# IntelLabs/GKL

Hardware: AMD Instinct MI355X
Metric: pairhmm_gcups (higher is better)
Workload: dtype f32

## Files before the change

### gkl_amd/csrc/pairhmm_aux_kernels.h

```cpp
#pragma once
#include <hip/hip_runtime.h>
#include <stdint.h>

#include "../../include/gkl_hip_pairhmm.h"
#include "pairhmm_fwd_kernel.h"
#include "pairhmm_multi_sets.h"

namespace gklhip {

struct PrepArgs {
  const uint8_t* hap_bases;
  const int32_t* hap_src;
  const int32_t* hap_len;
  const int32_t* hap_pos;
  const int32_t* hap_group;
  const int32_t* hap_pos_flat;
  uint32_t* stream_flat;
  uint32_t* stream;
  uint8_t* hap_has_n;
  int32_t n_haps;
  int32_t* clear_a; int32_t n_a;
  int32_t* clear_b; int32_t n_b;
  int32_t* clear_c; int32_t n_c;
  const uint4* pull_src; uint4* pull_dst; int32_t pull_n16;
// ... 219 lines not shown
struct FinalizeArgs {
  const float* raw32;
  const double* raw64;
  double* out;
  uint8_t* used64;
  int32_t* count;
  int32_t* read_fail;
  int32_t n_haps;
  int64_t n;
  int mode;
  float log10_init_f;
  double log10_init32_as_f64;
  double log10_init_d;
};

__global__ void finalize32_kernel(FinalizeArgs a) {
  const int64_t i = (int64_t)blockIdx.x * blockDim.x + threadIdx.x;
  if (i >= a.n || a.used64[i]) return;
  const float v = a.raw32[i];
  if (a.mode == GKLHIP_FINALIZE_DEVICE_F64) a.out[i] = log10((double)v) - a.log10_init32_as_f64;
  else if (a.mode == GKLHIP_FINALIZE_DEVICE_REF32) a.out[i] = (double)((float)log10((double)v) - a.log10_init_f);
}

__global__ void finalize64_kernel(FinalizeArgs a, int all_pairs) {
  const int64_t p = (int64_t)blockIdx.x * blockDim.x + threadIdx.x;
  if (p >= a.n) return;
  if (all_pairs) a.used64[p] = 1;
  else if (!a.used64[p]) return;
  if (a.mode >= 0) a.out[p] = log10(a.raw64[p]) - a.log10_init_d;
  if (a.mode == kModePacked) reinterpret_cast<uint64_t*>(a.out)[p] = packed_word(a.raw64[p]);
}

#ifndef GKL_PACK_WINDOW
#define GKL_PACK_WINDOW 96
#endif
constexpr int kPackWindow = GKL_PACK_WINDOW;
// ... 13 lines not shown
  LaneSlot* lanes2;
  const int32_t* hap_orig;
  const int32_t* hap_group;
  const int32_t* hap_pos;
  const int32_t* hap_len;
  FwdJob* jobs;
  FwdJob* sorted;
  const LaneSlot* long_lanes;
  int32_t n_long;
  FwdJob* jobs_long;
  int32_t* long_chunk_jobs;
  int32_t total_cols;
  int32_t wanted_jobs;
  int32_t min_job_cols;
  int32_t packed_by_kernels;
};

__device__ __forceinline__ bool last_block_done(int32_t* arrivals) {
  __shared__ int32_t s_is_last;
  __syncthreads();
  if (threadIdx.x == 0) {
    __threadfence();
    const int32_t before = atomicAdd(arrivals, 1);
    s_is_last = before == (int32_t)gridDim.x - 1 ? 1 : 0;
    __threadfence();
  }
  __syncthreads();
  return s_is_last != 0;
}

__device__ __forceinline__ int32_t ld_cnt(int32_t* p) { return __hip_atomic_load(p, __ATOMIC_RELAXED, __HIP_MEMORY_SCOPE_AGENT); }

__device__ __forceinline__ int job_class(const FwdJob& j, const int32_t* hap_pos, const int32_t* hap_len) {
  const int cols = hap_pos[j.hap_end - 1] + hap_len[j.hap_end - 1] - hap_pos[j.hap_begin];
  const int c = cols >> 7;
  return kJobClasses - 1 - (c < kJobClasses - 1 ? c : kJobClasses - 1);
}

__device__ __forceinline__ void build_jobs_for_chunk(const PlanArgs& a, const LaneSlot* lanes, int c, FwdJob* jobs,
                                                     int32_t* chunk_jobs, int cut_cols, bool by_group, int lane) {
  const LaneSlot sl = lanes[(int64_t)c * kLanes + lane];
  jobs += (int64_t)c * a.n_haps;
  int n_jobs = 0;
  bool prev_need = false;
  uint64_t reads = __ballot(sl.read >= 0 && sl.block == 0);
  for (int k0 = 0; k0 < a.n_haps; k0 += kLanes) {
    const int k = k0 + lane;
    const bool in = k < a.n_haps;
    const int h = in ? a.hap_orig[k] : 0;
    uint8_t nd = 0;
    for (uint64_t m = reads; m; m &= m - 1) {
      const int r = __builtin_amdgcn_readlane(sl.read, __builtin_ctzll(m));
      if (in) nd |= a.fa.used64[(int64_t)r * a.n_haps + h];
    }
    const uint64_t need = __ballot(in && nd != 0);
    if (!need) { prev_need = false; continue; }
    bool start = false;
    if (in && nd) {
      const bool pred_needed = lane == 0 ? prev_need : ((need >> (lane - 1)) & 1ull) != 0;
      start = !pred_needed || a.hap_pos[k - 1] / cut_cols != a.hap_pos[k] / cut_cols ||
              (by_group && a.hap_group[k - 1] != a.hap_group[k]);
    }
    const uint64_t starts = __ballot(start);
    if ((need & 1ull) && !(starts & 1ull)) {
      const uint64_t stop = starts | ~need;
      const int e = stop ? __builtin_ctzll(stop) : kLanes;
      if (lane == 0) jobs[n_jobs - 1].hap_end = min(k0 + e, a.n_haps);
    }
    const int base = n_jobs;
    n_jobs += __builtin_popcountll(starts);
    if (start) {
      const uint64_t after = lane == kLanes - 1 ? 0ull : (~0ull << (lane + 1));
      const uint64_t stop = (starts | ~need) & after;
      const int e = stop ? __builtin_ctzll(stop) : kLanes;
      FwdJob j;
      j.chunk = c; j.hap_begin = k; j.hap_end = min(k0 + e, a.n_haps);
      j.klass = 0;
      jobs[base + __builtin_popcountll(starts & ((1ull << lane) - 1ull))] = j;
    }
    prev_need = ((need >> (kLanes - 1)) & 1ull) != 0;
  }
  __threadfence_block();
  for (int i = lane; i < n_jobs; i += kLanes) {
    FwdJob j = jobs[i];
    jobs[i].klass = job_class(j, a.hap_pos, a.hap_len);
  }
  if (lane == 0) chunk_jobs[c] = n_jobs;
}

#define GKLHIP_PLAN_STAMP(k) do { if (tid == 0) a.cnts[16 + (k)] = (int32_t)(wall_clock64() - clk0); } while (0)

constexpr int kPlanLdsBins = 4096;
template <bool kInLds>
__device__ __forceinline__ void order_affected_reads(const PlanArgs& a, int32_t* hist, int32_t* pos, int32_t* s_wave_tot,
                                                     int tid, uint64_t clk0) {
  constexpr int kBatch = 4;
  const int n = a.n_haps, lane = tid & 63, wave = tid >> 6;
  if (kInLds) {
    for (int c = tid; c < n + 2; c += kPlanBlock) hist[c] = 0;
    __syncthreads();
  }
// ... 73 lines not shown
      const bool fails = in_range && v < 1e-28f;
      const uint64_t mask = __ballot(fails);
      if (mask) {
        const int leader = __builtin_ctzll(mask);
        const int32_t read = fails ? (int32_t)((uint32_t)i / (uint32_t)a.n_haps) : -1;
        const int32_t lead_read = __shfl(read, leader, 64);
        const uint64_t same = __ballot(fails && read == lead_read);
        if (lane == leader) atomicAdd(a.fa.read_fail + lead_read, __builtin_popcountll(same));
        if (fails && read != lead_read) atomicAdd(a.fa.read_fail + read, 1);
        if (lane == 0) my_fails += __builtin_popcountll(mask);
      }
      if (in_range) {
        a.fa.used64[i] = fails ? 1 : 0;
        if (a.fa.mode == kModePacked && !a.packed_by_kernels)
          reinterpret_cast<uint64_t*>(a.fa.out)[i] = fails ? 0ull : (kPackedF32Tag | (uint64_t)__float_as_uint(v));
      }
    }
    if (lane == 0) s_wave[wave] = my_fails;
    __syncthreads();
    if (tid == 0) {
      int total = 0;
      for (int w = 0; w < kPlanBlock / 64; w++) total += s_wave[w];
      if (total) atomicAdd(a.cnts + 0, total);
    }
  }
  if (!last_block_done(a.cnts + 10)) return;
  const int n_fail = ld_cnt(a.cnts + 0);
  if (n_fail == 0) return;
  const uint64_t clk0 = wall_clock64();

  if (a.n_haps + 2 <= kPlanLdsBins) order_affected_reads<true>(a, s_hist, s_hist + kPlanLdsBins, s_i32, tid, clk0);
  else                             order_affected_reads<false>(a, a.hist, a.pos, s_i32, tid, clk0);
  GKLHIP_PLAN_STAMP(2);
}

__global__ __launch_bounds__(kPlanBlock) void plan_pack_kernel(PlanArgs a) {
  const int tid = (int)threadIdx.x, lane = tid & 63, wave = tid >> 6;
  const int nblk = (int)gridDim.x, blk = (int)blockIdx.x;
  if (ld_cnt(a.cnts + 0) == 0) return;
  const uint64_t clk0 = wall_clock64();

  {
    static_assert(kPackWindow <= 2 * kLanes, "the window's lane counts sit in two registers per lane");
    __shared__ int32_t s_pack[kPlanBlock / 64][4][kPackWindow];
    int32_t* s_read = s_pack[wave][0]; int32_t* s_needl = s_pack[wave][1]; int32_t* s_sread = s_pack[wave][2];
    int32_t* s_sneed = s_pack[wave][3];
    const int n = ld_cnt(a.cnts + 4);
    const int n_win = (n + kPackWindow - 1) / kPackWindow;
    for (int w = blk * (kPlanBlock / 64) + wave; w < n_win; w += nblk * (kPlanBlock / 64)) {
      const int w0 = w * kPackWindow;
      const int cnt = min(kPackWindow, n - w0);
      for (int i = lane; i < cnt; i += kLanes) {
        const int r = a.order[w0 + i];
        s_read[i] = r;
        s_needl[i] = (int)((a.read_off[r + 1] - a.read_off[r] + a.rpl) / a.rpl);
      }
      __builtin_amdgcn_wave_barrier();
      if (w == 0 && lane == 0) a.cnts[22] = (int32_t)(wall_clock64() - clk0);
      for (int i = lane; i < cnt; i += kLanes) {
        const int ni = s_needl[i];
        int rank = 0;
        for (int j = 0; j < cnt; j++) {
          const int nj = s_needl[j];
          rank += (nj > ni) || (nj == ni && j < i);
        }
        s_sread[rank] = s_read[i];
        s_sneed[rank] = ni;
      }
      __builtin_amdgcn_wave_barrier();
      if (w == 0 && lane == 0) a.cnts[23] = (int32_t)(wall_clock64() - clk0);
      int head = -1, next_lo = -1, next_hi = -1;
      int bin_lo = 0, off_lo = 0, bin_hi = 0, off_hi = 0;
      uint64_t avail = 0;
      int nb = 0;
      const int need_lo = lane < cnt ? s_sneed[lane] : 0, need_hi = lane + kLanes < cnt ? s_sneed[lane + kLanes] : 0;
      for (int i = 0; i < cnt; i++) {
        const int nn = __builtin_amdgcn_readlane(i < kLanes ? need_lo : need_hi, i & 63);
        const uint64_t fits = nn >= kLanes ? 0ull : (avail >> nn) << nn;
        int bin, f;
        if (fits) {
          f = __builtin_ctzll(fits);
          bin = __builtin_amdgcn_readlane(head, f);
          const int nxt = __builtin_amdgcn_readlane(bin < kLanes ? next_lo : next_hi, bin & 63);
          if (lane == f) head = nxt;
          if (nxt < 0) avail &= ~(1ull << f);
        } else {
          bin = nb++;
          f = kLanes;
        }
        const int left = f - nn;
        if (left > 0) {
          const int old = __builtin_amdgcn_readlane(head, left);
          if (lane == (bin & 63)) { if (bin < kLanes) next_lo = old; else next_hi = old; }
          if (lane == left) head = bin;
          avail |= 1ull << left;
        }
        if (lane == (i & 63)) { if (i < kLanes) { bin_lo = bin; off_lo = kLanes - f; } else { bin_hi = bin; off_hi = kLanes - f; } }
      }
      if (w == 0 && lane == 0) a.cnts[24] = (int32_t)(wall_clock64() - clk0);
      int base = 0;
      if (lane == 0) base = atomicAdd(a.cnts + 5, nb);
      base = __shfl(base, 0, kLanes);
      LaneSlot idle; idle.read = -1; idle.block = 0;
      for (int i = lane; i < nb * kLanes; i += kLanes) a.lanes2[(int64_t)base * kLanes + i] = idle;
      __builtin_amdgcn_wave_barrier();
      __threadfence_block();
      if (w == 0 && lane == 0) a.cnts[25] = (int32_t)(wall_clock64() - clk0);
      if (lane < cnt) {
        LaneSlot sl; sl.read = s_sread[lane];
        LaneSlot* dst = a.lanes2 + (int64_t)(base + bin_lo) * kLanes + off_lo;
        for (int b = 0; b < need_lo; b++) { sl.block = b; dst[b] = sl; }
      }
      if (lane + kLanes < cnt) {
        LaneSlot sl; sl.read = s_sread[lane + kLanes];
        LaneSlot* dst = a.lanes2 + (int64_t)(base + bin_hi) * kLanes + off_hi;
        for (int b = 0; b < need_hi; b++) { sl.block = b; dst[b] = sl; }
      }
      __builtin_amdgcn_wave_barrier();
      if (w == 0 && lane == 0) a.cnts[26] = (int32_t)(wall_clock64() - clk0);
    }
  }
  if (blk == 0) GKLHIP_PLAN_STAMP(3);
}

__global__ __launch_bounds__(kPlanBlock) void plan_jobs_kernel(PlanArgs a) {
  __shared__ int32_t s_i32[kPlanBlock];
  const int tid = (int)threadIdx.x, lane = tid & 63, wave = tid >> 6;
  const int nblk = (int)gridDim.x, blk = (int)blockIdx.x;
  const int n_fail = ld_cnt(a.cnts + 0);
  if (n_fail == 0) return;
  const uint64_t clk0 = wall_clock64();

  {
    const int total = ld_cnt(a.cnts + 5);
    const int n_fail_reads = ld_cnt(a.cnts + 4);
    const double density = (double)n_fail / ((double)max(n_fail_reads, 1) * (double)a.n_haps);
    const double est_steps = (double)max(total, 1) * (double)a.total_cols * fmin(density, 1.0);
    const int cut_cols = max(a.min_job_cols, (int)fmin(est_steps / (double)a.wanted_jobs, 1e9));
    const int n_waves = nblk * (kPlanBlock / 64), w = blk * (kPlanBlock / 64) + wave;
    for (int c = w; c < total; c += n_waves) build_jobs_for_chunk(a, a.lanes2, c, a.jobs, a.order, cut_cols, false, lane);
    for (int c = w; c < a.n_long; c += n_waves) build_jobs_for_chunk(a, a.long_lanes, c, a.jobs_long, a.long_chunk_jobs, 0x7fffffff, true, lane);
  }
  if (!last_block_done(a.cnts + 11)) return;
  GKLHIP_PLAN_STAMP(4);

  {
    int32_t* cnt = s_i32;
    int32_t* base = s_i32 + kJobClasses;
    const int total = ld_cnt(a.cnts + 5);
    __syncthreads();
    if (tid < kJobClasses) cnt[tid] = 0;
    __syncthreads();
    for (int c = tid; c < total; c += kPlanBlock) {
      const FwdJob* mine = a.jobs + (int64_t)c * a.n_haps;
      const int n = a.order[c];
      for (int i = 0; i < n; i++) atomicAdd(&cnt[mine[i].klass], 1);
    }
    __syncthreads();
    if (tid == 0) {
      int acc = 0;
      for (int c = 0; c < kJobClasses; c++) { base[c] = acc; acc += cnt[c]; }
      a.cnts[2] = acc;
    }
    __syncthreads();
    for (int c = tid; c < total; c += kPlanBlock) {
      const FwdJob* mine = a.jobs + (int64_t)c * a.n_haps;
      const int n = a.order[c];
      for (int i = 0; i < n; i++) {
        const FwdJob j = mine[i];
        a.sorted[atomicAdd(&base[j.klass], 1)] = j;
      }
    }
    if (tid == 0 && a.n_long > 0) {
      int at = 0;
      for (int c = 0; c < a.n_long; c++) {
        const int n = a.long_chunk_jobs[c];
        for (int i = 0; i < n; i++) a.jobs_long[at++] = a.jobs_long[(int64_t)c * a.n_haps + i];
      }
      a.cnts[8] = at;
    }
  }
  GKLHIP_PLAN_STAMP(5);
}
#undef GKLHIP_PLAN_STAMP

// ... 223 lines not shown
```

### gkl_amd/csrc/pairhmm_ctx.h

```cpp
#pragma once

using namespace gklhip;

namespace {
struct EnvSwitches {
  static bool on_unless_zero(const char* name) { const char* v = getenv(name); return !v || atoi(v) != 0; }
  static int integer(const char* name) { const char* v = getenv(name); return v ? atoi(v) : 0; }
  const bool wide_long = on_unless_zero("GKLHIP_WIDE_LONG");
  const bool super_long = on_unless_zero("GKLHIP_SUPER_LONG");
  const bool fused_pairs = on_unless_zero("GKLHIP_FUSED_PAIRS");
  const int64_t fused_max = [] { const char* v = getenv("GKLHIP_FUSED_MAX_PAIRS"); return v ? atoll(v) : -1LL; }();
  const bool xcd_aware = on_unless_zero("GKLHIP_XCD_AWARE");
  const bool timing = getenv("GKLHIP_TIMING") != nullptr;
  const int combine_load = integer("GKL_HIP_COMBINE_LOAD");
  const int target_cols = integer("GKLHIP_TARGET_COLS");
  const int fb_wanted_jobs = integer("GKLHIP_FB_WANTED_JOBS");
  const int plan_blocks = integer("GKLHIP_PLAN_BLOCKS");
  const int finalize_threads = integer("GKL_HIP_FINALIZE_THREADS");
  const int finalize_min = integer("GKL_HIP_FINALIZE_MIN");
  const bool combine = [] { const char* v = getenv("GKL_HIP_COMBINE"); return !(v && v[0] == '0'); }();
  const bool combine_mid = integer("GKL_HIP_COMBINE_MID") != 0;
  const bool quiet = getenv("GKL_HIP_QUIET") != nullptr;
  const bool one_device_engine = integer("GKL_HIP_DEVICE_ENGINES") == 1;
  const int small_read_limit = integer("GKL_HIP_SMALL_READ_LIMIT") == 511 ? 511 : 383;
// ... 21 lines not shown
  PinBuf stage_slot[2];
  DevBuf plan_dev_slot[2];
  hipEvent_t stage_free_slot[2] = {nullptr, nullptr};
  hipEvent_t plan_unused_slot[2] = {nullptr, nullptr};
  hipStream_t upload_stream = nullptr;
  bool upload_eager = false;
  hipStream_t pad_stream = nullptr;
  int plan_slot = 0;
  DevBuf raw32, raw64, used64, counters, stream_buf, out_dev;
  DevBuf lanes_main;
  DevBuf read_fail, lanes2, jobs, jobs_long, fail_order, fail_hist, hap_flags;
  DevBuf batch_dev;
  PinBuf res_pin;
  WorkerPool workers;
  hipStream_t copy_stream = nullptr;
  hipEvent_t policy_done = nullptr, early_copy_done = nullptr;
  hipEvent_t call_done = nullptr;
  bool have_call_done = false;
  static constexpr int kEventRing = 64;
  hipEvent_t ev_ring[kEventRing][6] = {};
  hipEvent_t* ev = ev_ring[0];
  int64_t calls = 0;
  bool ring_double[kEventRing] = {};
  gklhip_stats stats;
  int64_t last_pairs = 0;
  hipStream_t last_stream = nullptr;
  bool have_last = false;
  Plan plan;
  std::vector<PlanLane> long_lanes;
  std::vector<FwdJob> long_jobs;
  DevBuf carry;
// ... 4 lines not shown
```

### gkl_amd/csrc/pairhmm_ctx_lifecycle.h

```cpp
#pragma once

namespace {

std::atomic<int> g_eager_upload_holders{0};

int trim_streams(DevCtx* c) {
  if (!c->copy_stream && !c->pad_stream && (!c->upload_stream || c->upload_eager)) return 0;
  (void)hipSetDevice(c->device);
  for (hipStream_t s : {c->stream, c->copy_stream, c->upload_stream, c->have_last ? c->last_stream : nullptr})
    if (s && hipStreamQuery(s) != hipSuccess) { (void)hipGetLastError(); return 0; }
  int n = 0;
  if (c->copy_stream) { (void)hipStreamDestroy(c->copy_stream); c->copy_stream = nullptr; n++; }
  if (c->pad_stream) { (void)hipStreamDestroy(c->pad_stream); c->pad_stream = nullptr; n++; }
  if (c->upload_stream && !c->upload_eager) { (void)hipStreamDestroy(c->upload_stream); c->upload_stream = nullptr; n++; }
  return n;
}

void dev_done(DevCtx* c) {
  if (!c) return;
  (void)hipSetDevice(c->device);
  if (c->upload_eager) g_eager_upload_holders--;
  if (c->stream) (void)hipStreamSynchronize(c->stream);
  if (c->last_stream && c->have_last) (void)hipStreamSynchronize(c->last_stream);
  for (DevBuf* b : {&c->tab32, &c->tab64, &c->plan_dev_slot[0], &c->plan_dev_slot[1], &c->raw32, &c->raw64, &c->used64,
                    &c->counters, &c->stream_buf, &c->out_dev, &c->batch_dev, &c->read_fail, &c->lanes_main,
                    &c->lanes2, &c->jobs, &c->jobs_long, &c->fail_order, &c->fail_hist, &c->carry, &c->hap_flags})
    b->release();
  c->stage_slot[0].release();
  c->stage_slot[1].release();
  c->res_pin.release();
  c->multi_fallbacks.release();
  if (c->multi_in) (void)hipEventDestroy(c->multi_in);
  if (c->policy_done) (void)hipEventDestroy(c->policy_done);
  if (c->early_copy_done) (void)hipEventDestroy(c->early_copy_done);
  if (c->call_done) (void)hipEventDestroy(c->call_done);
  if (c->copy_stream) { (void)hipStreamSynchronize(c->copy_stream); (void)hipStreamDestroy(c->copy_stream); }
  for (auto& set : c->ev_ring)
    for (auto& e : set) if (e) (void)hipEventDestroy(e);
  for (int k = 0; k < 2; k++) {
    if (c->stage_free_slot[k]) (void)hipEventDestroy(c->stage_free_slot[k]);
    if (c->plan_unused_slot[k]) (void)hipEventDestroy(c->plan_unused_slot[k]);
  }
  if (c->upload_stream) { (void)hipStreamSynchronize(c->upload_stream); (void)hipStreamDestroy(c->upload_stream); }
  if (c->pad_stream) (void)hipStreamDestroy(c->pad_stream);
  if (c->stream) (void)hipStreamDestroy(c->stream);
  delete c;
}

int dev_init(const gklhip_config& cfg, int dev, int ndev, DevCtx** out) {
// ... 73 lines not shown
    if (hipStreamCreateWithFlags(&c->upload_stream, hipStreamNonBlocking) != hipSuccess) { g_eager_upload_holders--; return bail(fail(GKLHIP_ERR_HIP, "hipStreamCreate failed")); }
    c->upload_eager = true;
  } else {
    g_eager_upload_holders--;
  }
  if (const char* v = getenv("GKL_HIP_EAGER_STREAMS")) {
    const int k = atoi(v);
    if (k >= 7) { if (aux_streams(c) != GKLHIP_OK) return bail(GKLHIP_ERR_HIP); }
    else for (int i = 0; i < k; i++) { hipStream_t d = nullptr; (void)hipStreamCreateWithFlags(&d, hipStreamNonBlocking); }
  }
  for (int k = 0; k < 2; k++)
    if (hipEventCreateWithFlags(&c->stage_free_slot[k], hipEventDisableTiming) != hipSuccess ||
        hipEventCreateWithFlags(&c->plan_unused_slot[k], hipEventDisableTiming) != hipSuccess)
      return bail(fail(GKLHIP_ERR_HIP, "hipEventCreate failed"));
  if (hipEventCreateWithFlags(&c->policy_done, hipEventDisableTiming) != hipSuccess ||
      hipEventCreateWithFlags(&c->early_copy_done, hipEventDisableTiming) != hipSuccess ||
      hipEventCreateWithFlags(&c->call_done, hipEventDisableTiming) != hipSuccess)
    return bail(fail(GKLHIP_ERR_HIP, "hipEventCreate failed"));
  for (int k = 0; k < 2; k++)
    if (hipEventRecord(c->stage_free_slot[k], c->stream) != hipSuccess || hipEventRecord(c->plan_unused_slot[k], c->stream) != hipSuccess)
      return bail(fail(GKLHIP_ERR_HIP, "hipEventRecord failed"));
  {
    const int sets = c->cfg.record_events == 2 ? DevCtx::kEventRing : 1;
    for (int k = 0; k < sets; k++)
      for (auto& e : c->ev_ring[k])
        if (hipEventCreate(&e) != hipSuccess) return bail(fail(GKLHIP_ERR_HIP, "hipEventCreate failed"));
  }
  if ((rc = upload_tables(c, host_tables_f32(), &c->tab32, &c->dt32))) return bail(rc);
  if ((rc = upload_tables(c, host_tables_f64(), &c->tab64, &c->dt64))) return bail(rc);
  *out = c;
  return GKLHIP_OK;
// ... 42 lines not shown
```

### gkl_amd/csrc/pairhmm_device_pass.h

```cpp
#pragma once

namespace {

int aux_streams(DevCtx* c) {
  if (!c->upload_stream) HIP_TRY(hipStreamCreateWithFlags(&c->upload_stream, hipStreamNonBlocking));
  if (!c->copy_stream) {
    HIP_TRY(hipStreamCreateWithFlags(&c->copy_stream, hipStreamNonBlocking));
    if (!c->pad_stream) HIP_TRY(hipStreamCreateWithFlags(&c->pad_stream, hipStreamNonBlocking));
  }
  return GKLHIP_OK;
}

template <typename T>
int upload_tables(DevCtx* c, const HostTables<T>& h, DevBuf* buf, DevTables<T>* dt) {
  const size_t n = (size_t)kQuals * 2 + kMmEntries;
  int st = buf->reserve(n * sizeof(T));
  if (st) return st;
  T* base = buf->as<T>();
  {
    T* pin = nullptr;
    HIP_TRY(hipHostMalloc(reinterpret_cast<void**>(&pin), n * sizeof(T), hipHostMallocDefault));
    memcpy(pin, h.ph2pr.data(), kQuals * sizeof(T));
    memcpy(pin + kQuals, h.div3.data(), kQuals * sizeof(T));
    memcpy(pin + 2 * kQuals, h.mm.data(), kMmEntries * sizeof(T));
// ... 135 lines not shown
};

#ifndef GKL_RPL_F64
#define GKL_RPL_F64 6
#endif
constexpr int kRplF64 = GKL_RPL_F64;
#ifndef GKL_RPL_F64_JOBS
#define GKL_RPL_F64_JOBS 10
#endif
constexpr int kRplF64Jobs = GKL_RPL_F64_JOBS;
constexpr int kRplF64Wide = 8;
constexpr size_t kSmallBatchBytes = 1 << 20;
constexpr int64_t kDirectPairs = 65536;
constexpr int64_t kTwoStepFrom = 2048;
constexpr int64_t kSmallDoublePairs = kTwoStepFrom;
constexpr int kPlanBlocks = 64;
constexpr int kFallbackWantedJobs = 12288;
constexpr int64_t kHostShardPairs = 400000;
constexpr int64_t kOnePassPairs = 65536;
constexpr int kTargetCols = 2048;
#ifndef GKL_RPL_F32
#define GKL_RPL_F32 8
#endif
constexpr int kRplF32 = GKL_RPL_F32;
std::atomic<int> g_host_calls_in_flight{0};
int pick_f32_rpl(int forced, int n_reads, int n_haps, const int64_t* read_off, const int64_t* hap_off, int load = 1) {
  int max_len = 0;
  for (int r = 0; r < n_reads; r++) max_len = std::max(max_len, (int)(read_off[r + 1] - read_off[r]));
  if (forced == 2 && max_len <= 2 * kLanes - 1) return 2;
  if (forced == 4 || forced == -4 || forced == 2) return 4;
  if (forced == 8) return kRplF32;
// ... 299 lines not shown
  } else {
    if ((rc = aux_streams(c))) return rc;
    HIP_TRY(hipStreamWaitEvent(c->upload_stream, c->plan_unused_slot[slot], 0));
    HIP_TRY(hipMemcpyAsync(dp, hs, L.total, hipMemcpyHostToDevice, c->upload_stream));
    HIP_TRY(hipEventRecord(c->stage_free_slot[slot], c->upload_stream));
    HIP_TRY(hipStreamWaitEvent(s, c->stage_free_slot[slot], 0));
  }
  if (g_env.timing)
    fprintf(stderr, "[gklhip] host plan + staging: %.3f ms (%d chunks, %d stream entries, %zu plan bytes)\n",
            std::chrono::duration<double, std::milli>(std::chrono::steady_clock::now() - P.t0).count(),
            plan.n_chunks, plan.n_stream, L.total);

  if ((rc = c->raw32.reserve((size_t)P.n_pairs * 4))) return rc;
  if ((rc = c->raw64.reserve((size_t)P.n_pairs * 8))) return rc;
  if ((rc = c->used64.reserve((size_t)P.n_pairs))) return rc;
  if ((rc = c->counters.reserve(128))) return rc;
  if ((rc = c->read_fail.reserve((size_t)P.n_reads * 4))) return rc;
  if ((rc = c->stream_buf.reserve(((size_t)plan.n_stream + (size_t)plan.n_stream_flat) * 4))) return rc;
  if (!P.use_double && (rc = c->fail_hist.reserve((size_t)P.n_hist * 4))) return rc;
  if ((rc = c->hap_flags.reserve((size_t)P.n_haps))) return rc;
  if ((rc = c->lanes_main.reserve((size_t)std::max(plan.n_chunks, 1) * kLanes * sizeof(LaneSlot)))) return rc;

  S.s = s; S.out = out_dev; S.slot = slot; S.hs = hs; S.dp = dp; S.xcarry = nullptr;
  const gklhip_batch dbi = P.inline_host() ? batch_at(*db, dp + L.batch, L.batch_stride) : *db;
  S.b = DevBatch{dbi.read_bases, dbi.read_quals, dbi.ins_gop, dbi.del_gop, dbi.gcp, reinterpret_cast<const int64_t*>(dp + L.read_off), P.n_reads, P.n_haps};
  S.hap_bases = (P.pull && P.inline_host()) ? batch_at(*db, S.hs_dev + L.batch, L.batch_stride).hap_bases : dbi.hap_bases;
  S.stream_grouped = P.inline_host() ? reinterpret_cast<uint32_t*>(dp + L.stream) : c->stream_buf.as<uint32_t>();
  S.stream_flat = P.inline_host() ? reinterpret_cast<uint32_t*>(dp + L.stream_flat) : c->stream_buf.as<uint32_t>() + plan.n_stream;
  S.hap_has_n = P.inline_host() ? dp + L.has_n : c->hap_flags.as<uint8_t>();
  return GKLHIP_OK;
}
// ... 117 lines not shown
  pa.lanes2 = c->lanes2.as<LaneSlot>();
  pa.hap_orig = reinterpret_cast<const int32_t*>(dp + L.hap_orig);
  pa.hap_group = reinterpret_cast<const int32_t*>(dp + L.hap_group);
  pa.hap_pos = reinterpret_cast<const int32_t*>(dp + L.hap_pos_flat);
  pa.hap_len = reinterpret_cast<const int32_t*>(dp + L.hap_len);
  pa.jobs = c->jobs.as<FwdJob>();
  pa.sorted = c->jobs.as<FwdJob>() + planned_max_jobs(P);
  pa.long_lanes = reinterpret_cast<const LaneSlot*>(dp + L.long_lanes) + (size_t)P.n_long_main * kLanes;
  pa.n_long = P.n_long64;
  pa.jobs_long = c->jobs_long.as<FwdJob>();
  pa.long_chunk_jobs = c->fail_order.as<int32_t>() + n_reads;
  pa.total_cols = (int32_t)std::min<int64_t>((int64_t)P.hl + n_haps, 0x7fffffff);
  pa.wanted_jobs = g_env.fb_wanted_jobs > 0 ? g_env.fb_wanted_jobs : (int)std::min<int64_t>(kFallbackWantedJobs, std::max<int64_t>(4096, P.n_pairs / 100));
  pa.min_job_cols = 256;
  pa.packed_by_kernels = (P.finalize_mode == kModePacked && !P.per_pair) ? 1 : 0;
  return pa;
}

int launch_prep(DevCtx* c, const CallPlan& P, const StagedCall& S) {
  const bool ev = c->cfg.record_events != 0;
  if (ev) {
    const bool deferred = c->cfg.record_events == 2;
    c->ev = c->ev_ring[deferred ? c->calls % DevCtx::kEventRing : 0];
    c->ring_double[deferred ? c->calls % DevCtx::kEventRing : 0] = P.use_double;
    c->calls++;
    HIP_TRY(hipEventRecord(c->ev[0], S.s));
  }
  const PrepArgs pa = prep_args(c, P, S);
  hipLaunchKernelGGL(prep_kernel, dim3((unsigned)prep_grid(pa, P)), dim3(kPrepBlock), 0, S.s, pa);
  if (P.pull) HIP_TRY(hipEventRecord(c->stage_free_slot[S.slot], S.s));
// ... 51 lines not shown
int launch_planned_fp64(DevCtx* c, const CallPlan& P, const StagedCall& S) {
  const bool ev = c->cfg.record_events != 0;
  hipStream_t s = S.s;
  const int n_reads = P.n_reads;
  const int64_t n_pairs = P.n_pairs;
  const size_t max_jobs = planned_max_jobs(P);
  int rc;
  if ((rc = c->fail_order.reserve(((size_t)n_reads + (size_t)P.n_long64) * 4))) return rc;
  if ((rc = c->lanes2.reserve((size_t)n_reads * kLanes * sizeof(LaneSlot)))) return rc;
  if ((rc = c->jobs.reserve(2 * max_jobs * sizeof(FwdJob)))) return rc;
  if (P.n_long64 > 0 && (rc = c->jobs_long.reserve((size_t)P.n_long64 * (size_t)P.n_haps * sizeof(FwdJob)))) return rc;
  const PlanArgs pa = plan_args(c, P, S);
  const int blocks_env = g_env.plan_blocks;
  const int policy_grid = std::max(1, blocks_env > 0 ? blocks_env : (int)std::min<int64_t>(c->n_cus, std::max<int64_t>(16, n_pairs / 4096)));
  const int64_t max_windows = ((int64_t)n_reads + kPackWindow - 1) / kPackWindow;
  const int pack_grid = (int)std::max<int64_t>(1, std::min<int64_t>(kPlanBlocks, (max_windows + kPlanBlock / 64 - 1) / (kPlanBlock / 64)));
  const int jobs_grid = std::max(1, std::min(c->n_cus, blocks_env > 0 ? blocks_env : (int)std::min<int64_t>(kPlanBlocks, std::max<int64_t>(16, n_pairs / 8192))));
  hipLaunchKernelGGL(plan_policy_kernel, dim3((unsigned)policy_grid), dim3(kPlanBlock), 0, s, pa);
  HIP_TRY(hipEventRecord(c->policy_done, s));
  hipLaunchKernelGGL(plan_pack_kernel, dim3((unsigned)pack_grid), dim3(kPlanBlock), 0, s, pa);
  hipLaunchKernelGGL(plan_jobs_kernel, dim3((unsigned)jobs_grid), dim3(kPlanBlock), 0, s, pa);
  const bool side_finalize = finalizes_on_device(P.finalize_mode);
  if (side_finalize) {
    if ((rc = aux_streams(c))) return rc;
    HIP_TRY(hipStreamWaitEvent(c->copy_stream, c->policy_done, 0));
    hipLaunchKernelGGL(finalize32_kernel, dim3((unsigned)((n_pairs + 255) / 256)), dim3(256), 0, c->copy_stream, pa.fa);
    HIP_TRY(hipEventRecord(c->early_copy_done, c->copy_stream));
  }
  FwdArgs<double> d = recompute_args(c, P, S);
  d.chunk_lanes = c->lanes2.as<LaneSlot>();
  d.n_chunks = n_reads;
  d.jobs = c->jobs.as<FwdJob>() + max_jobs;
  if (ev) HIP_TRY(hipEventRecord(c->ev[3], s));
  launch_jobs<double, kRplF64Jobs>(d, P.fma, (int)std::min<int64_t>(n_pairs, (int64_t)c->n_cus * 16), s);
  if (P.n_long64 > 0) {
    int32_t* cnts = c->counters.as<int32_t>();
    FwdArgs<double> ld = d;
    ld.chunk_lanes = pa.long_lanes;
    ld.jobs = c->jobs_long.as<FwdJob>();
    ld.job_count = cnts + 8;
    ld.job_next = cnts + 9;
    launch_long_jobs<double, kRplF64Wide, kRplF64>(ld, P.fma, P.n_long_waves, c->plan.max_read_len, c->carry.as<double>(), P.carry_len, s, S.xcarry, P.xsteps, cnts + 13);
  }
  if (ev) HIP_TRY(hipEventRecord(c->ev[4], s));
  hipLaunchKernelGGL(finalize64_kernel, dim3((unsigned)((n_pairs + 255) / 256)), dim3(256), 0, s, pa.fa, 0);
  if (side_finalize) HIP_TRY(hipStreamWaitEvent(s, c->early_copy_done, 0));
  return GKLHIP_OK;
}
int finish_call(DevCtx* c, const CallPlan& P, const StagedCall& S) {
  const bool ev = c->cfg.record_events != 0;
  hipStream_t s = S.s;
  gklhip_stats& st = c->stats;
  if (ev) HIP_TRY(hipEventRecord(c->ev[5], s));
  HIP_TRY(hipGetLastError());

  HIP_TRY(hipEventRecord(c->plan_unused_slot[S.slot], s));
  HIP_TRY(hipEventRecord(c->call_done, s));
  c->have_call_done = true;
  c->last_pairs = P.n_pairs;
  c->last_stream = s;
  c->have_last = true;

  if (ev && c->cfg.record_events != 2) {
    HIP_TRY(hipEventSynchronize(c->ev[5]));
    float ms = 0;
    HIP_TRY(hipEventElapsedTime(&ms, c->ev[1], c->ev[2])); st.ms_fwd_main = ms;
    HIP_TRY(hipEventElapsedTime(&ms, c->ev[3], c->ev[4])); st.ms_fwd_fallback = P.use_double ? 0.f : ms;
    HIP_TRY(hipEventElapsedTime(&ms, c->ev[0], c->ev[5])); st.ms_total_device = ms;
    int32_t cnt[2] = {0, 0};
    HIP_TRY(hipMemcpyAsync(cnt, c->counters.p, 8, hipMemcpyDeviceToHost, s));
    HIP_TRY(hipStreamSynchronize(s));
    st.n_fallback = P.use_double ? P.n_pairs : cnt[0];
    if (g_env.timing && !P.use_double) {
      int32_t k[32];
      HIP_TRY(hipMemcpy(k, c->counters.p, sizeof k, hipMemcpyDeviceToHost));
      fprintf(stderr, "[gklhip] policy+plan phases, each from the start of its own launch (us): hist %.1f scan %.1f scatter %.1f pack %.1f jobs %.1f sort %.1f | "
              "%d affected reads, %d chunks, %d jobs | window 0: loaded %.1f ranked %.1f fitted %.1f cleared %.1f written %.1f\n",
              k[16] * 0.01, k[17] * 0.01, k[18] * 0.01, k[19] * 0.01, k[20] * 0.01, k[21] * 0.01,
              k[4], k[5], k[2], k[22] * 0.01, k[23] * 0.01, k[24] * 0.01, k[25] * 0.01, k[26] * 0.01);
    }
  } else {
    st.n_fallback = P.use_double ? P.n_pairs : -1;
  }
  return GKLHIP_OK;
}

int32_t small_call_kind(const CallPlan& P) {
  if (P.use_double && P.n_pairs > kSmallDoublePairs) return kSmallDoubleStream;
  return P.pair_double ? kSmallDouble : P.fused ? kSmallFused : P.n_pairs > kTwoStepFrom ? kSmallTwoStep : kSmallOneLaunch;
}
bool small_kind_is_mid(int32_t kind) { return kind == kSmallTwoStep || kind == kSmallDoubleStream; }

void describe_small_call(DevCtx* c, const CallPlan& P, const StagedCall& S, SmallLaunch* out) {
  SmallCall& k = out->call;
// ... 49 lines not shown
```

Before: 4669.

## Fuse f32 finalize into policy kernel and restructure fallback planning kernels

Drops the separate finalize32 kernel and its side stream, event wait and pass over the pairs by writing the f32 log10 result inside the policy kernel. Job classes are now computed as each job is stored and counted per block, so the jobs kernel merges per-block class counts instead of re-reading every job to build a histogram. The pack kernel moves to 256-thread blocks with a larger grid, ranks two window entries per lane, and makes bin placement branch-free. It also batches the flag reads in build_jobs and the job loads in the scatter, at the cost of more code complexity and an extra per-block counter buffer.

```diff
diff --git a/gkl_amd/csrc/pairhmm_aux_kernels.h b/gkl_amd/csrc/pairhmm_aux_kernels.h
--- a/gkl_amd/csrc/pairhmm_aux_kernels.h
+++ b/gkl_amd/csrc/pairhmm_aux_kernels.h
@@ -257,12 +257,9 @@
   double log10_init_d;
 };
 
-__global__ void finalize32_kernel(FinalizeArgs a) {
-  const int64_t i = (int64_t)blockIdx.x * blockDim.x + threadIdx.x;
-  if (i >= a.n || a.used64[i]) return;
-  const float v = a.raw32[i];
-  if (a.mode == GKLHIP_FINALIZE_DEVICE_F64) a.out[i] = log10((double)v) - a.log10_init32_as_f64;
-  else if (a.mode == GKLHIP_FINALIZE_DEVICE_REF32) a.out[i] = (double)((float)log10((double)v) - a.log10_init_f);
+__device__ __forceinline__ double finalize32_value(const FinalizeArgs& a, float v) {
+  if (a.mode == GKLHIP_FINALIZE_DEVICE_F64) return log10((double)v) - a.log10_init32_as_f64;
+  return (double)((float)log10((double)v) - a.log10_init_f);
 }
 
 __global__ void finalize64_kernel(FinalizeArgs a, int all_pairs) {
@@ -306,6 +303,7 @@
   int32_t wanted_jobs;
   int32_t min_job_cols;
   int32_t packed_by_kernels;
+  int32_t* class_part;
 };
 
 __device__ __forceinline__ bool last_block_done(int32_t* arrivals) {
@@ -323,60 +321,95 @@
 
 __device__ __forceinline__ int32_t ld_cnt(int32_t* p) { return __hip_atomic_load(p, __ATOMIC_RELAXED, __HIP_MEMORY_SCOPE_AGENT); }
 
-__device__ __forceinline__ int job_class(const FwdJob& j, const int32_t* hap_pos, const int32_t* hap_len) {
-  const int cols = hap_pos[j.hap_end - 1] + hap_len[j.hap_end - 1] - hap_pos[j.hap_begin];
+__device__ __forceinline__ int job_class(int cols) {
   const int c = cols >> 7;
   return kJobClasses - 1 - (c < kJobClasses - 1 ? c : kJobClasses - 1);
 }
+__device__ __forceinline__ void store_job(FwdJob* at, int chunk, int hap_begin, int hap_end, int cols, int32_t* s_class) {
+  FwdJob j;
+  j.chunk = chunk; j.hap_begin = hap_begin; j.hap_end = hap_end;
+  j.klass = job_class(cols);
+  *at = j;
+  if (s_class) atomicAdd(s_class + j.klass, 1);
+}
 
 __device__ __forceinline__ void build_jobs_for_chunk(const PlanArgs& a, const LaneSlot* lanes, int c, FwdJob* jobs,
-                                                     int32_t* chunk_jobs, int cut_cols, bool by_group, int lane) {
+                                                     int32_t* chunk_jobs, int cut_cols, bool by_group, int lane, int32_t* s_class) {
   const LaneSlot sl = lanes[(int64_t)c * kLanes + lane];
   jobs += (int64_t)c * a.n_haps;
   int n_jobs = 0;
   bool prev_need = false;
-  uint64_t reads = __ballot(sl.read >= 0 && sl.block == 0);
+  int open_at = -1, open_begin = 0, open_end = 0, open_pos = 0, open_pos_end = 0;
+  const uint64_t reads = __ballot(sl.read >= 0 && sl.block == 0);
+  const int n_chunk_reads = __builtin_popcountll(reads);
+  int my_read = 0;
+  {
+    int i = 0;
+    for (uint64_t m = reads; m; m &= m - 1, i++) {
+      const int r = __builtin_amdgcn_readlane(sl.read, __builtin_ctzll(m));
+      if (lane == i) my_read = r;
+    }
+  }
   for (int k0 = 0; k0 < a.n_haps; k0 += kLanes) {
     const int k = k0 + lane;
     const bool in = k < a.n_haps;
-    const int h = in ? a.hap_orig[k] : 0;
+    const int kc = min(k, a.n_haps - 1), kb = max(kc - 1, 0);
+    const int h = a.hap_orig[kc];
+    const int pos = a.hap_pos[kc];
+    const int pos_end = pos + a.hap_len[kc];
+    const int pos_before = a.hap_pos[kb];
+    const bool new_group = by_group && a.hap_group[kb] != a.hap_group[kc];
+    const uint8_t* flags = a.fa.used64 + h;
     uint8_t nd = 0;
-    for (uint64_t m = reads; m; m &= m - 1) {
-      const int r = __builtin_amdgcn_readlane(sl.read, __builtin_ctzll(m));
-      if (in) nd |= a.fa.used64[(int64_t)r * a.n_haps + h];
+    for (int i0 = 0; i0 < n_chunk_reads; i0 += 4) {
+      uint8_t v[4];
+#pragma unroll
+      for (int u = 0; u < 4; u++) {
+        const int r = __builtin_amdgcn_readlane(my_read, min(i0 + u, n_chunk_reads - 1));
+        v[u] = flags[(int64_t)r * a.n_haps];
+      }
+      nd |= v[0] | v[1] | v[2] | v[3];
     }
     const uint64_t need = __ballot(in && nd != 0);
-    if (!need) { prev_need = false; continue; }
     bool start = false;
     if (in && nd) {
       const bool pred_needed = lane == 0 ? prev_need : ((need >> (lane - 1)) & 1ull) != 0;
-      start = !pred_needed || a.hap_pos[k - 1] / cut_cols != a.hap_pos[k] / cut_cols ||
-              (by_group && a.hap_group[k - 1] != a.hap_group[k]);
+      start = !pred_needed || pos_before / cut_cols != pos / cut_cols || new_group;
     }
     const uint64_t starts = __ballot(start);
-    if ((need & 1ull) && !(starts & 1ull)) {
-      const uint64_t stop = starts | ~need;
-      const int e = stop ? __builtin_ctzll(stop) : kLanes;
-      if (lane == 0) jobs[n_jobs - 1].hap_end = min(k0 + e, a.n_haps);
+    if (open_at >= 0) {
+      bool ends = true;
+      if ((need & 1ull) && !(starts & 1ull)) {
+        const uint64_t stop = starts | ~need;
+        open_end = min(k0 + (stop ? __builtin_ctzll(stop) : kLanes), a.n_haps);
+        open_pos_end = __builtin_amdgcn_readlane(pos_end, open_end - 1 - k0);
+        ends = stop != 0;
+      }
+      if (ends) {
+        if (lane == 0) store_job(jobs + open_at, c, open_begin, open_end, open_pos_end - open_pos, s_class);
+        open_at = -1;
+      }
     }
     const int base = n_jobs;
     n_jobs += __builtin_popcountll(starts);
-    if (start) {
-      const uint64_t after = lane == kLanes - 1 ? 0ull : (~0ull << (lane + 1));
-      const uint64_t stop = (starts | ~need) & after;
-      const int e = stop ? __builtin_ctzll(stop) : kLanes;
-      FwdJob j;
-      j.chunk = c; j.hap_begin = k; j.hap_end = min(k0 + e, a.n_haps);
-      j.klass = 0;
-      jobs[base + __builtin_popcountll(starts & ((1ull << lane) - 1ull))] = j;
+    const uint64_t after = lane == kLanes - 1 ? 0ull : (~0ull << (lane + 1));
+    const uint64_t stop = (starts | ~need) & after;
+    const int hap_end = min(k0 + (stop ? __builtin_ctzll(stop) : kLanes), a.n_haps);
+    const int last_pos_end = __shfl(pos_end, hap_end - 1 - k0, kLanes);
+    const bool opens = start && !stop && k0 + kLanes < a.n_haps;
+    const int at = base + __builtin_popcountll(starts & ((1ull << lane) - 1ull));
+    if (start && !opens) store_job(jobs + at, c, k, hap_end, last_pos_end - pos, s_class);
+    const uint64_t opened = __ballot(opens);
+    if (opened) {
+      const int l = __builtin_ctzll(opened);
+      open_at = __builtin_amdgcn_readlane(at, l);
+      open_begin = k0 + l; open_end = k0 + kLanes;
+      open_pos = __builtin_amdgcn_readlane(pos, l);
+      open_pos_end = __builtin_amdgcn_readlane(pos_end, kLanes - 1);
     }
     prev_need = ((need >> (kLanes - 1)) & 1ull) != 0;
   }
-  __threadfence_block();
-  for (int i = lane; i < n_jobs; i += kLanes) {
-    FwdJob j = jobs[i];
-    jobs[i].klass = job_class(j, a.hap_pos, a.hap_len);
-  }
+  if (open_at >= 0 && lane == 0) store_job(jobs + open_at, c, open_begin, open_end, open_pos_end - open_pos, s_class);
   if (lane == 0) chunk_jobs[c] = n_jobs;
 }
 
@@ -480,6 +513,8 @@
         a.fa.used64[i] = fails ? 1 : 0;
         if (a.fa.mode == kModePacked && !a.packed_by_kernels)
           reinterpret_cast<uint64_t*>(a.fa.out)[i] = fails ? 0ull : (kPackedF32Tag | (uint64_t)__float_as_uint(v));
+        if (!fails && (a.fa.mode == GKLHIP_FINALIZE_DEVICE_F64 || a.fa.mode == GKLHIP_FINALIZE_DEVICE_REF32))
+          a.fa.out[i] = finalize32_value(a.fa, v);
       }
     }
     if (lane == 0) s_wave[wave] = my_fails;
@@ -500,69 +535,70 @@
   GKLHIP_PLAN_STAMP(2);
 }
 
-__global__ __launch_bounds__(kPlanBlock) void plan_pack_kernel(PlanArgs a) {
-  const int tid = (int)threadIdx.x, lane = tid & 63, wave = tid >> 6;
+constexpr int kPackBlock = 256;
+__global__ __launch_bounds__(kPackBlock) void plan_pack_kernel(PlanArgs a) {
+  const int tid = (int)threadIdx.x, lane = tid & 63, wave = __builtin_amdgcn_readfirstlane(tid >> 6);
   const int nblk = (int)gridDim.x, blk = (int)blockIdx.x;
   if (ld_cnt(a.cnts + 0) == 0) return;
   const uint64_t clk0 = wall_clock64();
 
   {
     static_assert(kPackWindow <= 2 * kLanes, "the window's lane counts sit in two registers per lane");
-    __shared__ int32_t s_pack[kPlanBlock / 64][4][kPackWindow];
+    __shared__ int32_t s_pack[kPackBlock / 64][4][kPackWindow];
     int32_t* s_read = s_pack[wave][0]; int32_t* s_needl = s_pack[wave][1]; int32_t* s_sread = s_pack[wave][2];
     int32_t* s_sneed = s_pack[wave][3];
-    const int n = ld_cnt(a.cnts + 4);
+    const int n = __builtin_amdgcn_readfirstlane(ld_cnt(a.cnts + 4));
     const int n_win = (n + kPackWindow - 1) / kPackWindow;
-    for (int w = blk * (kPlanBlock / 64) + wave; w < n_win; w += nblk * (kPlanBlock / 64)) {
+    for (int w = blk * (kPackBlock / 64) + wave; w < n_win; w += nblk * (kPackBlock / 64)) {
       const int w0 = w * kPackWindow;
       const int cnt = min(kPackWindow, n - w0);
       for (int i = lane; i < cnt; i += kLanes) {
         const int r = a.order[w0 + i];
         s_read[i] = r;
-        s_needl[i] = (int)((a.read_off[r + 1] - a.read_off[r] + a.rpl) / a.rpl);
+        s_needl[i] = ((int)(a.read_off[r + 1] - a.read_off[r]) + a.rpl) / a.rpl;
       }
       __builtin_amdgcn_wave_barrier();
       if (w == 0 && lane == 0) a.cnts[22] = (int32_t)(wall_clock64() - clk0);
-      for (int i = lane; i < cnt; i += kLanes) {
-        const int ni = s_needl[i];
-        int rank = 0;
+      {
+        const int n_lo = lane < cnt ? s_needl[lane] : 0, n_hi = lane + kLanes < cnt ? s_needl[lane + kLanes] : 0;
+        int rank_lo = 0, rank_hi = 0;
+#pragma unroll 4
         for (int j = 0; j < cnt; j++) {
           const int nj = s_needl[j];
-          rank += (nj > ni) || (nj == ni && j < i);
+          rank_lo += (nj > n_lo) || (nj == n_lo && j < lane);
+          rank_hi += (nj > n_hi) || (nj == n_hi && j < lane + kLanes);
         }
-        s_sread[rank] = s_read[i];
-        s_sneed[rank] = ni;
+        if (lane < cnt) { s_sread[rank_lo] = s_read[lane]; s_sneed[rank_lo] = n_lo; }
+        if (lane + kLanes < cnt) { s_sread[rank_hi] = s_read[lane + kLanes]; s_sneed[rank_hi] = n_hi; }
       }
       __builtin_amdgcn_wave_barrier();
       if (w == 0 && lane == 0) a.cnts[23] = (int32_t)(wall_clock64() - clk0);
       int head = -1, next_lo = -1, next_hi = -1;
-      int bin_lo = 0, off_lo = 0, bin_hi = 0, off_hi = 0;
       uint64_t avail = 0;
       int nb = 0;
       const int need_lo = lane < cnt ? s_sneed[lane] : 0, need_hi = lane + kLanes < cnt ? s_sneed[lane + kLanes] : 0;
-      for (int i = 0; i < cnt; i++) {
-        const int nn = __builtin_amdgcn_readlane(i < kLanes ? need_lo : need_hi, i & 63);
+      auto place = [&](int nn) {
         const uint64_t fits = nn >= kLanes ? 0ull : (avail >> nn) << nn;
-        int bin, f;
-        if (fits) {
-          f = __builtin_ctzll(fits);
-          bin = __builtin_amdgcn_readlane(head, f);
-          const int nxt = __builtin_amdgcn_readlane(bin < kLanes ? next_lo : next_hi, bin & 63);
-          if (lane == f) head = nxt;
-          if (nxt < 0) avail &= ~(1ull << f);
-        } else {
-          bin = nb++;
-          f = kLanes;
-        }
+        const bool has = fits != 0;
+        const int f = has ? __builtin_ctzll(fits) : kLanes;
+        const int top = __builtin_amdgcn_readlane(head, f & 63);
+        const int bin = has ? top : nb;
+        nb += has ? 0 : 1;
+        const int nxt = __builtin_amdgcn_readlane(top < kLanes ? next_lo : next_hi, top & 63);
+        if (lane == f) head = nxt;
+        avail &= ~((uint64_t)(has && nxt < 0) << (f & 63));
         const int left = f - nn;
-        if (left > 0) {
-          const int old = __builtin_amdgcn_readlane(head, left);
-          if (lane == (bin & 63)) { if (bin < kLanes) next_lo = old; else next_hi = old; }
-          if (lane == left) head = bin;
-          avail |= 1ull << left;
-        }
-        if (lane == (i & 63)) { if (i < kLanes) { bin_lo = bin; off_lo = kLanes - f; } else { bin_hi = bin; off_hi = kLanes - f; } }
-      }
+        const bool keep = left > 0;
+        const int old = __builtin_amdgcn_readlane(head, left);
+        if (keep && lane == (bin & 63)) { if (bin < kLanes) next_lo = old; else next_hi = old; }
+        if (keep && lane == left) head = bin;
+        avail |= (uint64_t)keep << left;
+        return (bin << 8) | (kLanes - f);
+      };
+      int at_lo = 0, at_hi = 0;
+      for (int i = 0; i < min(cnt, kLanes); i++) { const int at = place(__builtin_amdgcn_readlane(need_lo, i)); if (lane == i) at_lo = at; }
+      for (int i = kLanes; i < cnt; i++) { const int at = place(__builtin_amdgcn_readlane(need_hi, i - kLanes)); if (lane == i - kLanes) at_hi = at; }
+      const int bin_lo = at_lo >> 8, off_lo = at_lo & 255, bin_hi = at_hi >> 8, off_hi = at_hi & 255;
       if (w == 0 && lane == 0) a.cnts[24] = (int32_t)(wall_clock64() - clk0);
       int base = 0;
       if (lane == 0) base = atomicAdd(a.cnts + 5, nb);
@@ -585,56 +621,71 @@
       __builtin_amdgcn_wave_barrier();
       if (w == 0 && lane == 0) a.cnts[26] = (int32_t)(wall_clock64() - clk0);
     }
+    if (lane == 0) atomicMax(a.cnts + 27, (int32_t)(wall_clock64() - clk0));
   }
   if (blk == 0) GKLHIP_PLAN_STAMP(3);
 }
 
 __global__ __launch_bounds__(kPlanBlock) void plan_jobs_kernel(PlanArgs a) {
-  __shared__ int32_t s_i32[kPlanBlock];
-  const int tid = (int)threadIdx.x, lane = tid & 63, wave = tid >> 6;
+  __shared__ int32_t s_i32[2 * kJobClasses];
+  const int tid = (int)threadIdx.x, lane = tid & 63, wave = __builtin_amdgcn_readfirstlane(tid >> 6);
   const int nblk = (int)gridDim.x, blk = (int)blockIdx.x;
-  const int n_fail = ld_cnt(a.cnts + 0);
+  const int n_fail = __builtin_amdgcn_readfirstlane(ld_cnt(a.cnts + 0));
   if (n_fail == 0) return;
   const uint64_t clk0 = wall_clock64();
+  int32_t* cnt = s_i32;
+  int32_t* base = s_i32 + kJobClasses;
+  if (tid < 2 * kJobClasses) s_i32[tid] = 0;
+  __syncthreads();
+
+  {
+    const int total = __builtin_amdgcn_readfirstlane(ld_cnt(a.cnts + 5));
+    const int n_fail_reads = __builtin_amdgcn_readfirstlane(ld_cnt(a.cnts + 4));
+    const double density = (double)n_fail / ((double)max(n_fail_reads, 1) * (double)a.n_haps);
+    const double est_steps = (double)max(total, 1) * (double)a.total_cols * fmin(density, 1.0);
+    const int cut_cols = __builtin_amdgcn_readfirstlane(max(a.min_job_cols, (int)fmin(est_steps / (double)a.wanted_jobs, 1e9)));
+    const int n_waves = nblk * (kPlanBlock / 64), w = blk * (kPlanBlock / 64) + wave;
+    for (int c = w; c < total; c += n_waves) build_jobs_for_chunk(a, a.lanes2, c, a.jobs, a.order, cut_cols, false, lane, cnt);
+    for (int c = w; c < a.n_long; c += n_waves) build_jobs_for_chunk(a, a.long_lanes, c, a.jobs_long, a.long_chunk_jobs, 0x7fffffff, true, lane, nullptr);
+  }
+  __syncthreads();
+  if (tid < kJobClasses) a.class_part[blk * kJobClasses + tid] = cnt[tid];
+  if (!last_block_done(a.cnts + 11)) return;
+  GKLHIP_PLAN_STAMP(4);
 
   {
     const int total = ld_cnt(a.cnts + 5);
-    const int n_fail_reads = ld_cnt(a.cnts + 4);
-    const double density = (double)n_fail / ((double)max(n_fail_reads, 1) * (double)a.n_haps);
-    const double est_steps = (double)max(total, 1) * (double)a.total_cols * fmin(density, 1.0);
-    const int cut_cols = max(a.min_job_cols, (int)fmin(est_steps / (double)a.wanted_jobs, 1e9));
-    const int n_waves = nblk * (kPlanBlock / 64), w = blk * (kPlanBlock / 64) + wave;
-    for (int c = w; c < total; c += n_waves) build_jobs_for_chunk(a, a.lanes2, c, a.jobs, a.order, cut_cols, false, lane);
-    for (int c = w; c < a.n_long; c += n_waves) build_jobs_for_chunk(a, a.long_lanes, c, a.jobs_long, a.long_chunk_jobs, 0x7fffffff, true, lane);
-  }
-  if (!last_block_done(a.cnts + 11)) return;
-  GKLHIP_PLAN_STAMP(4);
-
-  {
-    int32_t* cnt = s_i32;
-    int32_t* base = s_i32 + kJobClasses;
-    const int total = ld_cnt(a.cnts + 5);
-    __syncthreads();
     if (tid < kJobClasses) cnt[tid] = 0;
     __syncthreads();
+    for (int i = tid; i < nblk * kJobClasses; i += kPlanBlock) {
+      const int n = a.class_part[i];
+      if (n) atomicAdd(&cnt[i & (kJobClasses - 1)], n);
+    }
+    __syncthreads();
+    if (wave == 0) {
+      static_assert(kJobClasses == 64, "one class per lane");
+      const int mine = cnt[lane];
+      int inc = mine;
+      for (int d = 1; d < 64; d <<= 1) {
+        const int o = __shfl_up(inc, d, 64);
+        if (lane >= d) inc += o;
+      }
+      base[lane] = inc - mine;
+      if (lane == 63) a.cnts[2] = inc;
+    }
+    __syncthreads();
+    constexpr int kBatch = 4;
     for (int c = tid; c < total; c += kPlanBlock) {
       const FwdJob* mine = a.jobs + (int64_t)c * a.n_haps;
       const int n = a.order[c];
-      for (int i = 0; i < n; i++) atomicAdd(&cnt[mine[i].klass], 1);
-    }
-    __syncthreads();
-    if (tid == 0) {
-      int acc = 0;
-      for (int c = 0; c < kJobClasses; c++) { base[c] = acc; acc += cnt[c]; }
-      a.cnts[2] = acc;
-    }
-    __syncthreads();
-    for (int c = tid; c < total; c += kPlanBlock) {
-      const FwdJob* mine = a.jobs + (int64_t)c * a.n_haps;
-      const int n = a.order[c];
-      for (int i = 0; i < n; i++) {
-        const FwdJob j = mine[i];
-        a.sorted[atomicAdd(&base[j.klass], 1)] = j;
+      for (int i0 = 0; i0 < n; i0 += kBatch) {
+        FwdJob j[kBatch];
+#pragma unroll
+        for (int k = 0; k < kBatch; k++)
+          if (i0 + k < n) j[k] = mine[i0 + k];
+#pragma unroll
+        for (int k = 0; k < kBatch; k++)
+          if (i0 + k < n) a.sorted[atomicAdd(&base[j[k].klass], 1)] = j[k];
       }
     }
     if (tid == 0 && a.n_long > 0) {
diff --git a/gkl_amd/csrc/pairhmm_ctx.h b/gkl_amd/csrc/pairhmm_ctx.h
--- a/gkl_amd/csrc/pairhmm_ctx.h
+++ b/gkl_amd/csrc/pairhmm_ctx.h
@@ -59,7 +59,7 @@
   PinBuf res_pin;
   WorkerPool workers;
   hipStream_t copy_stream = nullptr;
-  hipEvent_t policy_done = nullptr, early_copy_done = nullptr;
+  hipEvent_t policy_done = nullptr;
   hipEvent_t call_done = nullptr;
   bool have_call_done = false;
   static constexpr int kEventRing = 64;
diff --git a/gkl_amd/csrc/pairhmm_ctx_lifecycle.h b/gkl_amd/csrc/pairhmm_ctx_lifecycle.h
--- a/gkl_amd/csrc/pairhmm_ctx_lifecycle.h
+++ b/gkl_amd/csrc/pairhmm_ctx_lifecycle.h
@@ -32,7 +32,6 @@
   c->multi_fallbacks.release();
   if (c->multi_in) (void)hipEventDestroy(c->multi_in);
   if (c->policy_done) (void)hipEventDestroy(c->policy_done);
-  if (c->early_copy_done) (void)hipEventDestroy(c->early_copy_done);
   if (c->call_done) (void)hipEventDestroy(c->call_done);
   if (c->copy_stream) { (void)hipStreamSynchronize(c->copy_stream); (void)hipStreamDestroy(c->copy_stream); }
   for (auto& set : c->ev_ring)
@@ -136,7 +135,6 @@
         hipEventCreateWithFlags(&c->plan_unused_slot[k], hipEventDisableTiming) != hipSuccess)
       return bail(fail(GKLHIP_ERR_HIP, "hipEventCreate failed"));
   if (hipEventCreateWithFlags(&c->policy_done, hipEventDisableTiming) != hipSuccess ||
-      hipEventCreateWithFlags(&c->early_copy_done, hipEventDisableTiming) != hipSuccess ||
       hipEventCreateWithFlags(&c->call_done, hipEventDisableTiming) != hipSuccess)
     return bail(fail(GKLHIP_ERR_HIP, "hipEventCreate failed"));
   for (int k = 0; k < 2; k++)
diff --git a/gkl_amd/csrc/pairhmm_device_pass.h b/gkl_amd/csrc/pairhmm_device_pass.h
--- a/gkl_amd/csrc/pairhmm_device_pass.h
+++ b/gkl_amd/csrc/pairhmm_device_pass.h
@@ -173,7 +173,10 @@
 constexpr int64_t kDirectPairs = 65536;
 constexpr int64_t kTwoStepFrom = 2048;
 constexpr int64_t kSmallDoublePairs = kTwoStepFrom;
-constexpr int kPlanBlocks = 64;
+constexpr int kPackBlocksMax = 256;
+constexpr int kPlanJobBlocks = 64;
+constexpr int kPlanJobBlocksMax = 256;
+constexpr size_t kCounterBytes = 128;
 constexpr int kFallbackWantedJobs = 12288;
 constexpr int64_t kHostShardPairs = 400000;
 constexpr int64_t kOnePassPairs = 65536;
@@ -503,7 +506,7 @@
   if ((rc = c->raw32.reserve((size_t)P.n_pairs * 4))) return rc;
   if ((rc = c->raw64.reserve((size_t)P.n_pairs * 8))) return rc;
   if ((rc = c->used64.reserve((size_t)P.n_pairs))) return rc;
-  if ((rc = c->counters.reserve(128))) return rc;
+  if ((rc = c->counters.reserve(kCounterBytes + (size_t)kPlanJobBlocksMax * kJobClasses * 4))) return rc;
   if ((rc = c->read_fail.reserve((size_t)P.n_reads * 4))) return rc;
   if ((rc = c->stream_buf.reserve(((size_t)plan.n_stream + (size_t)plan.n_stream_flat) * 4))) return rc;
   if (!P.use_double && (rc = c->fail_hist.reserve((size_t)P.n_hist * 4))) return rc;
@@ -651,6 +654,7 @@
   pa.wanted_jobs = g_env.fb_wanted_jobs > 0 ? g_env.fb_wanted_jobs : (int)std::min<int64_t>(kFallbackWantedJobs, std::max<int64_t>(4096, P.n_pairs / 100));
   pa.min_job_cols = 256;
   pa.packed_by_kernels = (P.finalize_mode == kModePacked && !P.per_pair) ? 1 : 0;
+  pa.class_part = c->counters.as<int32_t>() + kCounterBytes / 4;
   return pa;
 }
 
@@ -732,19 +736,12 @@
   const int blocks_env = g_env.plan_blocks;
   const int policy_grid = std::max(1, blocks_env > 0 ? blocks_env : (int)std::min<int64_t>(c->n_cus, std::max<int64_t>(16, n_pairs / 4096)));
   const int64_t max_windows = ((int64_t)n_reads + kPackWindow - 1) / kPackWindow;
-  const int pack_grid = (int)std::max<int64_t>(1, std::min<int64_t>(kPlanBlocks, (max_windows + kPlanBlock / 64 - 1) / (kPlanBlock / 64)));
-  const int jobs_grid = std::max(1, std::min(c->n_cus, blocks_env > 0 ? blocks_env : (int)std::min<int64_t>(kPlanBlocks, std::max<int64_t>(16, n_pairs / 8192))));
+  const int pack_grid = (int)std::max<int64_t>(1, std::min<int64_t>(kPackBlocksMax, (max_windows + kPackBlock / 64 - 1) / (kPackBlock / 64)));
+  const int jobs_grid = std::max(1, std::min(std::min(c->n_cus, kPlanJobBlocksMax), blocks_env > 0 ? blocks_env : (int)std::min<int64_t>(kPlanJobBlocks, std::max<int64_t>(16, n_pairs / 8192))));
   hipLaunchKernelGGL(plan_policy_kernel, dim3((unsigned)policy_grid), dim3(kPlanBlock), 0, s, pa);
-  HIP_TRY(hipEventRecord(c->policy_done, s));
-  hipLaunchKernelGGL(plan_pack_kernel, dim3((unsigned)pack_grid), dim3(kPlanBlock), 0, s, pa);
+  if (!finalizes_on_device(P.finalize_mode)) HIP_TRY(hipEventRecord(c->policy_done, s));
+  hipLaunchKernelGGL(plan_pack_kernel, dim3((unsigned)pack_grid), dim3(kPackBlock), 0, s, pa);
   hipLaunchKernelGGL(plan_jobs_kernel, dim3((unsigned)jobs_grid), dim3(kPlanBlock), 0, s, pa);
-  const bool side_finalize = finalizes_on_device(P.finalize_mode);
-  if (side_finalize) {
-    if ((rc = aux_streams(c))) return rc;
-    HIP_TRY(hipStreamWaitEvent(c->copy_stream, c->policy_done, 0));
-    hipLaunchKernelGGL(finalize32_kernel, dim3((unsigned)((n_pairs + 255) / 256)), dim3(256), 0, c->copy_stream, pa.fa);
-    HIP_TRY(hipEventRecord(c->early_copy_done, c->copy_stream));
-  }
   FwdArgs<double> d = recompute_args(c, P, S);
   d.chunk_lanes = c->lanes2.as<LaneSlot>();
   d.n_chunks = n_reads;
@@ -762,7 +759,6 @@
   }
   if (ev) HIP_TRY(hipEventRecord(c->ev[4], s));
   hipLaunchKernelGGL(finalize64_kernel, dim3((unsigned)((n_pairs + 255) / 256)), dim3(256), 0, s, pa.fa, 0);
-  if (side_finalize) HIP_TRY(hipStreamWaitEvent(s, c->early_copy_done, 0));
   return GKLHIP_OK;
 }
 int finish_call(DevCtx* c, const CallPlan& P, const StagedCall& S) {
@@ -793,9 +789,9 @@
       int32_t k[32];
       HIP_TRY(hipMemcpy(k, c->counters.p, sizeof k, hipMemcpyDeviceToHost));
       fprintf(stderr, "[gklhip] policy+plan phases, each from the start of its own launch (us): hist %.1f scan %.1f scatter %.1f pack %.1f jobs %.1f sort %.1f | "
-              "%d affected reads, %d chunks, %d jobs | window 0: loaded %.1f ranked %.1f fitted %.1f cleared %.1f written %.1f\n",
+              "%d affected reads, %d chunks, %d jobs | window 0: loaded %.1f ranked %.1f fitted %.1f cleared %.1f written %.1f, the last packing wavefront left after %.1f\n",
               k[16] * 0.01, k[17] * 0.01, k[18] * 0.01, k[19] * 0.01, k[20] * 0.01, k[21] * 0.01,
-              k[4], k[5], k[2], k[22] * 0.01, k[23] * 0.01, k[24] * 0.01, k[25] * 0.01, k[26] * 0.01);
+              k[4], k[5], k[2], k[22] * 0.01, k[23] * 0.01, k[24] * 0.01, k[25] * 0.01, k[26] * 0.01, k[27] * 0.01);
     }
   } else {
     st.n_fallback = P.use_double ? P.n_pairs : -1;
```

New measurement: 4690 (median of 2 runs). No clear change (+0.4%).
